# patour/distributed-membership

Hardware: AMD Instinct MI355X
Metric: simulated node-ticks/sec + achieved HBM GB/s at N=65,536 full-membership (higher is better)
Workload: dtype u8 cells (u16 escape lists) / 4-bit payload (integer)

## Files before the change

distributed-membership_amd/csrc/gm_band.h:

```cpp
#pragma once
#include "gm_device.h"
#include "gm_scaled.h"

template <int B>
struct RowMeta {
  int k;
  int snd[S_SB];
  uint32_t ebase;
  uint32_t bz;
  uint64_t evc;
  uint32_t ebase2, bz2;
  uint64_t evc2;
};

template <typename T>
__device__ __forceinline__ T gld(const T *p) {
#if __HIP_DEVICE_COMPILE__
  return *(const __attribute__((address_space(1))) T *)p;
#else
  return *p;
#endif
}
template <int B, bool UNI, bool EVC = false>
__device__ __forceinline__ RowMeta<B> row_meta(const SState &s, int r, int par, int t, size_t slab, int band,
                                               int band2 = -1) {
  RowMeta<B> m;
  const int rc = min(r, s.n - 1);
  const int32_t *ibase = par ? s.inbox[1] : s.inbox[0], *cbase = par ? s.inbox_cnt[1] : s.inbox_cnt[0];
  const int32_t *fbase = s.failed;
  const uint4 *rbase = s.brec;
  const uint64_t *ecbase = s.evcum;
  int ramp = s.ramp;
  if (UNI) asm("" : "+s"(ibase), "+s"(cbase), "+s"(fbase), "+s"(rbase), "+s"(ecbase), "+s"(ramp));
  const int32_t *ib = ibase + (size_t)rc * S_KMAX;
  const i32x4 av = gld((const i32x4 *)ib), bv = gld((const i32x4 *)(ib + 4));
  int4 a = make_int4(av.x, av.y, av.z, av.w);
  int4 b = make_int4(bv.x, bv.y, bv.z, bv.w);
  int k = gld(cbase + rc);
  int failed = gld(fbase + rc);
  const u32x4 rv = gld((const u32x4 *)(rbase + slab + rc));
  const uint4 rec = make_uint4(rv.x, rv.y, rv.z, rv.w);
  m.ebase = rec.w;
  m.bz = rec.z;
  m.evc = EVC ? gld(ecbase + (size_t)rc * s.nb + band) : 0ull;
  if (band2 >= 0) {
    const u32x4 rec2 = gld((const u32x4 *)(rbase + (size_t)band2 * s.n + rc));
    m.ebase2 = rec2.w;
    m.bz2 = rec2.z;
    m.evc2 = EVC ? gld(ecbase + (size_t)rc * s.nb + band2) : 0ull;
  }
  if (UNI) {
    asm volatile("" : "+s"(k), "+s"(failed), "+s"(a.x), "+s"(a.y), "+s"(a.z), "+s"(a.w));
    asm volatile("" : "+s"(b.x), "+s"(b.y), "+s"(b.z), "+s"(b.w));
  } else {
    asm volatile("" : "+v"(k), "+v"(failed));
  }
  m.snd[0] = a.x; m.snd[1] = a.y; m.snd[2] = a.z; m.snd[3] = a.w;
  m.snd[4] = b.x; m.snd[5] = b.y; m.snd[6] = b.z; m.snd[7] = b.w;
  m.k = (r >= s.n || failed || !s_ingroup(ramp, s.intro_until, r, t)) ? -1 : k;
  if (r >= s.n) m.ebase = m.ebase2 = 0;
  return m;
}

__device__ __forceinline__ void nib_max(u16x2 acc[8], uint32_t x0, uint32_t x1) {
  const u16x2 a = pk(x0), b = pk(x1);
  acc[0] = __builtin_elementwise_max(acc[0], a);
  acc[1] = __builtin_elementwise_max(acc[1], a << (u16x2)(4));
  acc[2] = __builtin_elementwise_max(acc[2], a << (u16x2)(8));
  acc[3] = __builtin_elementwise_max(acc[3], a << (u16x2)(12));
  acc[4] = __builtin_elementwise_max(acc[4], b);
  acc[5] = __builtin_elementwise_max(acc[5], b << (u16x2)(4));
  acc[6] = __builtin_elementwise_max(acc[6], b << (u16x2)(8));
  acc[7] = __builtin_elementwise_max(acc[7], b << (u16x2)(12));
}
__device__ __forceinline__ uint32_t nib_of(uint32_t x0, uint32_t x1, int q) {
  const uint32_t x = q < 8 ? x0 : x1;
  const int c = q & 7;
  return (x >> (16 * (c & 1) + 4 * (3 - (c >> 1)))) & 15u;
}
__device__ __forceinline__ uint32_t pesc_value(const SState &s, int pp, int band, int sn, int li, int q) {
  const uint4 rc = s.pesc_rec[pp][(size_t)band * s.n + sn];
  const uint64_t m = (uint64_t)rc.y | ((uint64_t)rc.z << 32);
  const uint32_t slot = rc.x + (uint32_t)__builtin_popcountll(m & ((1ull << li) - 1));
  return rc.x == S_PESC_NONE || slot >= s.pesc_cap ? 0u : (uint32_t)s.pesc[pp][(size_t)slot * 16 + q];
}
__device__ __forceinline__ uint32_t nib_value(uint32_t nb, const SState &s, int pp, int band, int sn, int li, int q) {
  return nb == S_NIB_ESC ? pesc_value(s, pp, band, sn, li, q) : nb ? S_NIB_H(nb) : 0u;
}

#define S_PHI 0x9E3779B9u
__device__ __forceinline__ uint32_t s_drop_pair(const SState &s, int t, int sn, int r) {
  return (uint32_t)gm_mix64(s.drop_seed ^ ((uint64_t)(uint32_t)(t - 1) << 48) ^ ((uint64_t)(uint32_t)sn << 24) ^
                            (uint64_t)(uint32_t)r);
}
__device__ __forceinline__ bool s_keep(const SState &s, int t, int sn, int r, int c, uint32_t T) {
  const uint32_t h = gm_fmix32(s_drop_pair(s, t, sn, r) ^ ((uint32_t)(c >> 1) * S_PHI));
  return ((h >> (16 * (c & 1))) & 0xFFFFu) >= T;
}
__device__ __forceinline__ constexpr int nib_pos(int q) { return 32 * (q >> 3) + 16 * (q & 1) + 4 * (3 - ((q & 7) >> 1)); }
__device__ __forceinline__ uint64_t s_keep_nibbles(const SState &s, int t, int sn, int r, int colb, uint32_t T,
                                                   bool agrp) {
  const uint32_t pair = s_drop_pair(s, t, sn, r);
  const int c = s.c0 + colb;
  if (T > 65535u) return 0;
  if (agrp) {
    const u16x2 t2 = (u16x2)((uint16_t)T);
    uint32_t kw[2] = {0u, 0u};
#pragma unroll
    for (int i = 0; i < 8; i++) {
      const uint32_t h = gm_fmix32(pair ^ ((uint32_t)((c >> 1) + i) * S_PHI));
      const u16x2 drop = pmin1(__builtin_elementwise_sub_sat(t2, pk(h)));
      kw[i >> 2] |= unpk(((u16x2)(1) - drop) * (u16x2)(0xFu << (4 * (3 - (i & 3)))));
    }
    return (uint64_t)kw[0] | ((uint64_t)kw[1] << 32);
  }
  uint64_t km = 0;
  for (int q = 0; q < 16; q++) {
    const uint32_t h = gm_fmix32(pair ^ ((uint32_t)((c + q) >> 1) * S_PHI));
    if (((h >> (16 * ((c + q) & 1))) & 0xFFFFu) >= T) km |= 0xFull << nib_pos(q);
  }
  return km;
}
__device__ __forceinline__ uint32_t nz_nibble_bits(uint32_t x) { return (x | (x >> 1) | (x >> 2) | (x >> 3)) & 0x11111111u; }

template <int B>
__device__ __forceinline__ void unit_table(const SState &s, UnitIn<B> &in) {
  constexpr int LPR = B / S_COLS_PER_LANE, Q = S_COLS_PER_LANE;
  const int li = (threadIdx.x & 63) % LPR;
  const __amdgpu_buffer_rsrc_t trs = gm_rsrc(s.table + (size_t)in.band * s.n * B, (uint32_t)(s.n * B));
  in.ta = __builtin_amdgcn_raw_buffer_load_b128(trs, (uint32_t)(in.r * B + li * Q), 0, GM_AUX_NT);
}

template <int B, bool UNI = false, bool EVC = false, bool TWO = false>
__device__ __forceinline__ void unit_load(const SState &s, int t, int band, int ub, UnitIn<B> &in,
                                          UnitIn<B> &in2, int band2) {
  constexpr int LPR = B / S_COLS_PER_LANE, RPW = 64 / LPR;
  const int sub = (threadIdx.x & 63) / LPR;
  in.band = band;
  in.r = ub * RPW + sub;
  in.msg = s.msg;
  in.tesc = (t & 1) ? s.tesc_in[0] : s.tesc_in[1];
  if (UNI) asm("" : "+s"(in.msg), "+s"(in.tesc));
  const size_t slab = (size_t)in.band * s.n;
  unit_table<B>(s, in);
  const RowMeta<B> meta = row_meta<B, UNI, EVC>(s, in.r, t & 1, t, slab, band, TWO ? band2 : -1);
#pragma unroll
  for (int j = 0; j < S_SB; j++) in.snd[j] = meta.snd[j];
  in.k = meta.k;
  in.ebase = meta.ebase;
  in.bz = meta.bz;
  in.evc = meta.evc;
  in.uni = EVC;
  if (TWO) {
    in2.band = band2;
    in2.r = in.r;
#pragma unroll
    for (int j = 0; j < S_SB; j++) in2.snd[j] = meta.snd[j];
    in2.k = meta.k;
    in2.ebase = meta.ebase2;
    in2.bz = meta.bz2;
    in2.evc = meta.evc2;
    in2.uni = EVC;
    in2.msg = in.msg;
    in2.tesc = in.tesc;
  }
}
template <int B, bool UNI = false, bool EVC = false>
__device__ __forceinline__ void unit_load(const SState &s, int t, int band, int ub, UnitIn<B> &in) {
  unit_load<B, UNI, EVC, false>(s, t, band, ub, in, in, -1);
}

template <int B, bool DROP>
__device__ __forceinline__ void unit_gather(const SState &s, int t, const UnitIn<B> &in, u32x2 m[S_SB], uint32_t &ent) {
  constexpr int LPR = B / S_COLS_PER_LANE;
  const int li = (threadIdx.x & 63) % LPR;
  ent = 0;
  if (li < (int)min(S_EW_TOT(in.ebase), (uint32_t)S_ESC_IN))
    ent = gld(in.tesc + ((size_t)in.band * s.n + in.r) * S_ESC_IN + li);
  const __amdgpu_buffer_rsrc_t prs = gm_rsrc(in.msg + (size_t)in.band * s.n * B, (uint32_t)(s.n * B));
  const uint32_t poff = (uint32_t)(((t & 1) ^ 1) * (B / 2) + li * 8);
  const int k = min(in.k, S_KMAX);
#pragma unroll
  for (int j = 0; j < S_SB; j++)
    m[j] = __builtin_amdgcn_raw_buffer_load_b64(prs, j < k ? poff + (uint32_t)in.snd[j] * B : GM_OOB, 0, 0);
}

struct RowCounts {
  uint64_t piece;
  int pf;
};
__device__ __forceinline__ RowCounts row_counts(int npres, int nfail) {
  int pf = npres | (nfail << 16);
  pf += __builtin_amdgcn_update_dpp(0, pf, 0xB1, 0xF, 0xF, false);
  pf += __builtin_amdgcn_update_dpp(0, pf, 0x4E, 0xF, 0xF, false);
  pf += __builtin_amdgcn_update_dpp(0, pf, 0x141, 0xF, 0xF, false);
  RowCounts rc;
  rc.piece = 0;
  rc.pf = 0;
#pragma unroll
  for (int c = 0; c < 8; c++) {
    const int v = __builtin_amdgcn_readlane(pf, 8 * c);
    rc.piece |= (uint64_t)(v & 0xFF) << (8 * c);
    rc.pf += v;
  }
  return rc;
}
template <int B, bool DROP>
__device__ __forceinline__ void unit_records(const SState &s, int t, const UnitIn<B> &in, bool live, uint32_t eb_out,
                                             int npres, int nfail, int nev, uint32_t evk, int nkept,
                                             const RowCounts *pre = nullptr) {
  constexpr int LPR = B / S_COLS_PER_LANE;
  constexpr int Q = S_COLS_PER_LANE;
  const int lane = threadIdx.x & 63;
  const int sub = lane / LPR, li = lane % LPR;
  const int band = in.band, r = in.r;
  const int colb = band * B + li * Q;
  const size_t slab = (size_t)band * s.n;
  if (DROP && s.mc_rdrop) {
    int v = nkept;
#pragma unroll
    for (int o = 1; o < LPR; o <<= 1) v += __shfl_xor(v, o, 64);
    if (live && li == 0 && v) atomicAdd(&s.mc_rdrop[r], (uint32_t)v);
  }
  constexpr int CH = S_CHUNK(B), LPC = CH / Q;
  int pf = npres | (nfail << 16);
  uint64_t piece = 0;
  if (LPR == 64 && LPC == 8 && pre) {
    piece = pre->piece;
    pf = pre->pf;
  } else if (LPR == 64 && LPC == 8) {
    const RowCounts rc = row_counts(npres, nfail);
    piece = rc.piece;
    pf = rc.pf;
  } else {
    int cc = npres;
#pragma unroll
    for (int o = 1; o < LPC; o <<= 1) cc += __shfl_xor(cc, o, 64);
#pragma unroll
    for (int c = 0; c < B / CH; c++) piece |= (uint64_t)(__shfl(cc, sub * LPR + LPC * c, 64) & 0xFF) << (8 * c);
#pragma unroll
    for (int o = LPR / 2; o >= 1; o >>= 1) pf += __shfl_xor(pf, o, 64);
  }
  int x = 0, tot = 0;
  if (__builtin_amdgcn_ballot_w64(nev != 0)) {
    int jr = __builtin_popcount(evk & 0x55555555u) | (__builtin_popcount(evk & 0xAAAAAAAAu) << 16);
    x = nev;
    if (LPR == 64) {
      x = dpp_scan(x);
      jr = dpp_scan(jr);
      tot = __builtin_amdgcn_readlane(x, 63);
      jr = __builtin_amdgcn_readlane(jr, 63);
    } else {
#pragma unroll
      for (int o = 1; o < LPR; o <<= 1) {
        const int y = __shfl_up(x, o, 64);
        if (li >= o) x += y;
      }
      tot = __shfl(x, sub * LPR + LPR - 1, 64);
#pragma unroll
      for (int o = LPR / 2; o >= 1; o >>= 1) jr += __shfl_xor(jr, o, 64);
    }
    if (live && li == 0 && jr) {
      const unsigned long long add = (unsigned long long)(jr & 0xFFFF) | ((unsigned long long)(jr >> 16) << 32);
      if (in.uni) s.evcum[(size_t)r * s.nb + band] = in.evc + add;
      else atomicAdd((unsigned long long *)&s.evcum[(size_t)r * s.nb + band], add);
    }
  }
  const int E = s.evs;
  uint32_t sbase = 0;
  if (live && li == 0 && tot > E) sbase = atomicAdd(s.ev_spill_cnt, (uint32_t)(tot - E));
  if (live && li == 0 && tot)
    atomicAdd(s.ev_spill_cnt + 1 + ((slab + (size_t)r) & (S_EV_STRIPES - 1)), (uint32_t)tot);
  sbase = LPR == 64 ? __builtin_amdgcn_readfirstlane(sbase) : __shfl(sbase, sub * LPR, 64);
  if (live && nev) {
    int slot = x - nev;
    uint32_t *slots = s.ev_band + ((size_t)r * s.nb + band) * E;
    for (uint32_t ek = evk; ek; ek &= ek - 1) {
      const int bit = __builtin_ctz(ek);
      const int q = bit >> 1;
      const uint32_t kind = (evk >> (2 * q)) & 3u;
      const uint32_t rec = (kind << 30) | (uint32_t)(s.c0 + colb + q + 1);
      if (slot < E) {
        slots[slot] = rec;
      } else {
        const uint32_t sp = sbase + (uint32_t)(slot - E);
        if (sp < s.ev_spill_cap) s.ev_spill[sp] = ((uint64_t)(uint32_t)r << 32) | rec;
        else atomicOr(s.err, GM_ERR_EVENTS);
      }
      slot++;
    }
  }
  if (li == 0 && r < s.n) {
    const uint32_t bc = (uint32_t)(pf & 0xFFFF) | ((uint32_t)(pf >> 16) << 11) | ((uint32_t)min(tot, 1023) << 22);
    s.brec[slab + r] = live ? make_uint4((uint32_t)piece, (uint32_t)(piece >> 32), bc, eb_out)
                            : make_uint4(0u, 0u, 0u, eb_out);
  }
}

template <int B, bool DROP>
__device__ __forceinline__ void unit_finish(const SState &s, int t, int drop_pct, const UnitIn<B> &in,
                                            const u32x2 m[S_SB], uint32_t ent, uint32_t *lds) {
  constexpr int LPR = B / S_COLS_PER_LANE;
  constexpr int RPW = 64 / LPR;
  constexpr int Q = S_COLS_PER_LANE;
  const int lane = threadIdx.x & 63;
  const int par = t & 1;
  const int sub = lane / LPR, li = lane % LPR;
  const int band = in.band, r = in.r;
  const int colb = band * B + li * Q;
  const size_t slab = (size_t)band * s.n;
  const __amdgpu_buffer_rsrc_t trs = gm_rsrc(s.table + slab * B, (uint32_t)(s.n * B));
  const __amdgpu_buffer_rsrc_t prs = gm_rsrc(s.msg + slab * B, (uint32_t)(s.n * B));
  const uint32_t toff = (uint32_t)(r * B + li * Q);
  const uint32_t poff = (uint32_t)((par ^ 1) * (B / 2) + li * 8);
  int k = in.k;
  if (k > S_KMAX) {
    if (li == 0) atomicOr(s.err, GM_ERR_INBOX);
    k = S_KMAX;
  }
  const bool live = k >= 0;
  const u32x4 ta = in.ta;
  struct {
    int snd[S_SB];
  } meta;
#pragma unroll
  for (int j = 0; j < S_SB; j++) meta.snd[j] = in.snd[j];
  int kw = 0;
  {
    const int kl = live ? k : 0;
#pragma unroll
    for (int w = 0; w < RPW; w++) kw = max(kw, __builtin_amdgcn_readlane(kl, w * LPR));
  }
  int npres = 0, nfail = 0, nev = 0;
  int nkept = 0;
  uint32_t evk = 0;
  bool esc_st = false;
  uint32_t eb_out = 0;
  if (!live && in.ebase != 0) {
    const int etot = (int)S_EW_TOT(in.ebase);
    eb_out = row_alloc<LPR>(s, par, slab, r, etot, li, lane);
    if (eb_out != 0) {
      const EscList src = esc_list(s, par ^ 1, slab, r, in.ebase), dst = esc_list(s, par, slab, r, eb_out);
      constexpr int P = LPR < S_ESC_IN ? LPR : S_ESC_IN;
      if (li < min(etot, P)) *dst.at(li) = ent;
      for (int i = P + li; i < etot; i += LPR) *dst.at(i) = *src.at(i);
    }
  }
  if (live) {
    const int32_t *ib = s.inbox[par] + (size_t)r * S_KMAX;
    u16x2 key5[8];
    {
      const uint32_t T = DROP ? s_drop_thresh(drop_pct) : 0u;
      const bool agrp = ((s.c0 + colb) & 1) == 0;
      u16x2 acc[8];
#pragma unroll
      for (int i = 0; i < 8; i++) acc[i] = (u16x2)(0);
      auto merge_list = [&](int sn, uint32_t x0, uint32_t x1) {
        if (DROP) {
          if (!(x0 | x1)) return;
          const uint64_t km = s_keep_nibbles(s, t, sn, r, colb, T, agrp);
          x0 &= (uint32_t)km;
          x1 &= (uint32_t)(km >> 32);
          if (s.mc_rdrop) nkept += __builtin_popcount(nz_nibble_bits(x0)) + __builtin_popcount(nz_nibble_bits(x1));
        }
        nib_max(acc, x0, x1);
      };
#pragma unroll
      for (int j = 0; j < S_SB; j++)
        if (j < kw) merge_list(meta.snd[j], m[j].x, m[j].y);
      for (int j = S_SB; j < k; j++) {
        const int sn = ib[j];
        const u32x2 mv = __builtin_amdgcn_raw_buffer_load_b64(prs, poff + (uint32_t)sn * B, 0, 0);
        merge_list(sn, mv.x, mv.y);
      }
      u16x2 nmax = (u16x2)(0);
#pragma unroll
      for (int i = 0; i < 8; i++) {
        const u16x2 nb = acc[i] >> (u16x2)(12);
        nmax = __builtin_elementwise_max(nmax, nb);
        key5[i] = pmin1(nb) * (u16x2)(S_NIB_BASE << 5) + nb * (u16x2)(64);
      }
      if (__builtin_elementwise_max(nmax.x, nmax.y) == S_NIB_ESC) {
#pragma unroll
        for (int i = 0; i < 8; i++) {
          const u16x2 nb = acc[i] >> (u16x2)(12);
#pragma unroll
          for (int h = 0; h < 2; h++) {
            if (nb[h] != S_NIB_ESC) continue;
            const int q = 2 * i + h;
            uint32_t kv = 0;
            for (int j = 0; j < k; j++) {
              const int sn = ib[j];
              if (DROP && !s_keep(s, t, sn, r, s.c0 + colb + q, T)) continue;
              const u32x2 mm = __builtin_amdgcn_raw_buffer_load_b64(prs, poff + (uint32_t)sn * B, 0, 0);
              kv = max(kv, nib_value(nib_of(mm.x, mm.y, q), s, par ^ 1, band, sn, li, q));
            }
            key5[i][h] = (uint16_t)(kv << 5);
          }
        }
      }
    }
    if (s.ramp && r == 0) {
#pragma unroll
      for (int q = 0; q < Q; q++) {
        const int c = s.c0 + colb + q;
        if (c >= 1 && colb + q < s.w && s_start(c) == t - 1) key5[q >> 1][q & 1] = (uint16_t)(255u << 5);
      }
    }
    const uint32_t tb4[4] = {ta.x, ta.y, ta.z, ta.w};
    u16x2 tw[8], npb = (u16x2)(0);
#pragma unroll
    for (int i = 0; i < 8; i++) {
      const u16x2 x = pk(byte_pair(tb4[i >> 1], i & 1));
      const u16x2 nz = pmin1(x);
      npb = padd(npb, nz);
      tw[i] = widen2(x, nz);
    }
    if (in.ebase != 0)
      esc_apply<LPR>(lds, lane, li, esc_list(s, par ^ 1, slab, r, in.ebase), (int)S_EW_TOT(in.ebase), ent, tw);
    u16x2 mm[8];
#pragma unroll
    for (int i = 0; i < 8; i++)
      mm[i] = __builtin_elementwise_max(__builtin_elementwise_sub_sat(tw[i], (u16x2)(63)), key5[i]);
    const int selfc = (r >= s.c0 && r < s.c0 + s.w) ? r - s.c0 - colb : -1;
    int selfapp = -1;
    if (selfc >= 0 && selfc < Q) {
      const int hb = s.hbctr[r] + 1;
      s.hbctr[r] = hb + 1;
      int tq = selfc;
      uint32_t selfcell = 0;
#pragma unroll
      for (int q = 0; q < Q; q++)
        if (q == selfc) selfcell = (unpk(mm[q >> 1]) >> (16 * (q & 1))) & 0xFFFFu;
      if (selfcell == 0) {
        if (!s.ramp) {
          atomicOr(s.err, GM_ERR_SELF);
        } else {
#pragma unroll
          for (int q = Q - 1; q >= 0; q--)
            if (q > selfc && q <= (selfc | 3) && ((unpk(mm[q >> 1]) >> (16 * (q & 1))) & 0xFFFFu)) tq = q;
          if (tq == selfc) {
            selfapp = selfc;
            const uint32_t slot = atomicAdd(s.selfadd_cnt, 1u);
            if (slot < S_SELFADD_CAP) s.selfadd[slot] = r;
            else atomicOr(s.err, GM_ERR_SELF);
            if (s.sharded) atomicOr((uint32_t *)(s.xcnt + S_XC(s, s.shard_rank, r)), S_XC_SELFAPP);
          }
        }
      }
      if (s.ramp) s.mecol[r] = s.c0 + colb + tq;
      const int h = 255 - (2 * t - (hb + s_hbase(s.ramp, s.c0 + colb + tq)));
      if (h < s.lag_hmin || h > 255) atomicOr(s.err, GM_ERR_LAG);
#pragma unroll
      for (int i = 0; i < 8; i++) {
        if ((tq >> 1) != i) continue;
        uint32_t v = unpk(mm[i]);
        const int sh = 16 * (tq & 1);
        v = (v & ~(0xFFFFu << sh)) | ((uint32_t)S_CELL(h, 0) << sh);
        mm[i] = pk(v);
      }
    }
    u16x2 np2 = (u16x2)(0), nf2 = (u16x2)(0), badv = (u16x2)(0), nmx = (u16x2)(0), amax = (u16x2)(0);
    u16x2 nwv[2] = {(u16x2)(0), (u16x2)(0)};
    uint32_t cw[8], bw[4];
    sweep_cells(mm, np2, nf2, badv, nmx, amax, nwv, cw, bw);
    int ngone = 0;
    uint32_t gmask = 0;
    if (__builtin_elementwise_max(amax.x, amax.y) >= GM_TREMOVE) {
      u16x2 ng2 = (u16x2)(0);
      uint32_t gprev = 0;
#pragma unroll
      for (int i = 0; i < 8; i++) {
        const u16x2 v = pk(cw[i]);
        const u16x2 gone = ((v & (u16x2)(31)) + (u16x2)(32 - GM_TREMOVE)) >> (u16x2)(5);
        gmask |= ((unpk(gone) & 1u) | ((unpk(gone) >> 15) & 2u)) << (2 * i);
        ng2 = padd(ng2, gone);
        const uint32_t gb = unpk(gone * (u16x2)(0xFF));
        if (i & 1) bw[i >> 1] &= ~__builtin_amdgcn_perm(gb, gprev, 0x06040200u);
        else gprev = gb;
      }
      np2 = np2 - ng2;
      ngone = (int)ng2.x + (int)ng2.y;
      badv = (u16x2)(esc_mask16(bw[0], bw[1], bw[2], bw[3]) != 0 ? 1 : 0);
    }
    esc_st = unpk(badv) != 0;
    const bool esc_row = row_any<LPR>(esc_st, sub);
    uint32_t em = 0;
    if (esc_row) {
      if (esc_st) {
        em = esc_mask16(bw[0], bw[1], bw[2], bw[3]);
        esc_park(lds, lane, cw);
      }
    }
    const bool pesc = __builtin_elementwise_max(nmx.x, nmx.y) == S_NIB_ESC;
    if (row_any<LPR>(pesc, sub)) payload_escapes<LPR>(s, par, slab, r, li, lane, sub, pesc, cw);
    nfail = (int)nf2.x + (int)nf2.y;
    npres = (int)np2.x + (int)np2.y;
    if (npres + ngone == (int)npb.x + (int)npb.y && ngone) {
      uint32_t x = gmask;
      x = (x | (x << 8)) & 0x00FF00FFu;
      x = (x | (x << 4)) & 0x0F0F0F0Fu;
      x = (x | (x << 2)) & 0x33333333u;
      x = (x | (x << 1)) & 0x55555555u;
      evk = x << 1;
      nev = __builtin_popcount(gmask);
    } else if (npres + ngone != (int)npb.x + (int)npb.y) {
      const u32x4 ra = __builtin_amdgcn_raw_buffer_load_b128(trs, toff, 0, 0);
      const uint32_t tb0[4] = {ra.x, ra.y, ra.z, ra.w};
#pragma unroll
      for (int q = 0; q < Q; q++) {
        const uint32_t before = (tb0[q >> 2] >> (8 * (q & 3))) & 0xFFu;
        const uint32_t after = (bw[q >> 2] >> (8 * (q & 3))) & 0xFFu;
        const uint32_t ev = !before ? (after && q != selfapp ? S_EV_ADD : 0u) : (!after ? S_EV_REMOVE : 0u);
        evk |= ev << (2 * q);
      }
      nev = __builtin_popcount((evk | (evk >> 1)) & 0x55555555u);
    }
    eb_out = unit_stores<B>(s, t, in, bw, unpk(nwv[0]), unpk(nwv[1]), esc_row, em, lds);
  }
  unit_records<B, DROP>(s, t, in, live, eb_out, npres, nfail, nev, evk, nkept);
}

__device__ __forceinline__ void band_reset_pools(const SState &s, int t) {
  const int S = s.esc_stripes;
  for (int i = threadIdx.x; i < S; i += 64) {
    s.tesc_cnt[((t & 1) ^ 1) * S + i] = 0;
    s.pesc_cnt[((t & 1) ^ 1) * S + i] = 0;
  }
  if (s.fb_cnt && threadIdx.x == 0) s.fb_cnt[(t & 1) ^ 1] = 0;
}

void gm_launch_selfcheck(const SState &s, hipStream_t st);
```

distributed-membership_amd/csrc/gm_band_fast.hip:

```cpp
#include "gm_band.h"

__device__ __forceinline__ int esc_bit(int q) { return ((q & 3) << 3) | (q >> 2); }
__device__ __forceinline__ int p_lanes_below(uint64_t b) {
  return (int)__builtin_amdgcn_mbcnt_hi((uint32_t)(b >> 32), __builtin_amdgcn_mbcnt_lo((uint32_t)b, 0u));
}
struct FastCell {
  uint32_t nbyte, nib, c;
  bool gone, bail;
  int dpres, dfail;
};
__device__ __forceinline__ FastCell fast_cell(const SState &s, int t, uint32_t y, uint32_t c, bool self, int hbself) {
  FastCell o;
  if (self) {
    if (c == 0) atomicOr(s.err, GM_ERR_SELF);
    const int h = 255 - (2 * t - hbself);
    if (h < s.lag_hmin || h > 255) atomicOr(s.err, GM_ERR_LAG);
    c = (uint32_t)S_CELL(h, 0) & 0xFFFFu;
  }
  const uint32_t age = c & 31u, h = c >> 5, hp = h - 2u;
  const bool pres = c != 0, stale = pres && age >= GM_TFAIL;
  o.gone = pres && age >= GM_TREMOVE;
  const bool keep = pres && !o.gone;
  const bool fits = h >= S_H4_MIN_H && !(h & 1u) && age <= S_AGE_MAX_B;
  o.nbyte = keep ? (fits ? ((((h - 224u) >> 1) << 4) | age) : S_B_ESC) : 0u;
  const bool fresh = keep && !stale;
  const bool nibok = !(hp & 1u) && hp >= S_NIB_H(1) && hp <= S_NIB_H(14);
  o.bail = fresh && !nibok;
  o.nib = fresh && nibok ? ((hp - S_NIB_BASE) >> 1) << 4 : 0u;
  o.c = c;
  const bool fpres = y >= 16u, fstale = fpres && (y & 15u) >= GM_TFAIL;
  o.dpres = (int)(pres && !o.gone) - (int)fpres;
  o.dfail = (int)stale - (int)fstale;
  return o;
}
template <int B, typename F>
__device__ __forceinline__ bool unit_fast(const SState &s, int t, const UnitIn<B> &in, const u32x2 m[S_SB],
                                          uint32_t ent, uint32_t *lds, uint32_t *park, F &&nxt) {
  static_assert(B / S_COLS_PER_LANE == 64, "the fast path takes one row per wave");
  constexpr int Q = S_COLS_PER_LANE;
  const int lane = threadIdx.x & 63, li = lane;
  const int par = t & 1;
  const int band = in.band, r = in.r;
  const int colb = band * B + li * Q;
  const size_t slab = (size_t)band * s.n;
  const int k = in.k;
  if (k > S_KMAX || s.ramp) return false;
  if (k < 0) {
    nxt();
    uint32_t eb_out = 0;
    if (in.ebase != 0) {
      const int etot = (int)S_EW_TOT(in.ebase);
      eb_out = row_alloc<64>(s, par, slab, r, etot, li, lane);
      if (eb_out != 0) {
        const EscList src = esc_list(s, par ^ 1, slab, r, in.ebase), dst = esc_list(s, par, slab, r, eb_out);
        if (li < min(etot, S_ESC_IN)) *dst.at(li) = ent;
        for (int i = S_ESC_IN + li; i < etot; i += 64) *dst.at(i) = *src.at(i);
      }
    }
    unit_records<B, false>(s, t, in, false, eb_out, 0, 0, 0, 0u, 0);
    return true;
  }
  u16x2 acc[8];
#pragma unroll
  for (int i = 0; i < 8; i++) acc[i] = (u16x2)(0);
#pragma unroll
  for (int j = 0; j < S_SB; j++)
    if (j < k) nib_max(acc, m[j].x, m[j].y);
  if (k > S_SB) {
    const __amdgpu_buffer_rsrc_t prs = gm_rsrc(s.msg + slab * B, (uint32_t)(s.n * B));
    const uint32_t poff = (uint32_t)((par ^ 1) * (B / 2) + li * 8);
    const int32_t *ib = s.inbox[par] + (size_t)r * S_KMAX;
    for (int j = S_SB; j < k; j++) {
      const int sn = ib[j];
      const u32x2 mv = __builtin_amdgcn_raw_buffer_load_b64(prs, poff + (uint32_t)sn * B, 0, 0);
      nib_max(acc, mv.x, mv.y);
    }
  }
  {
    u16x2 amx = acc[0];
#pragma unroll
    for (int i = 1; i < 8; i++) amx = __builtin_elementwise_max(amx, acc[i]);
    if (__builtin_amdgcn_ballot_w64(__builtin_elementwise_max(amx.x, amx.y) >= (uint16_t)(S_NIB_ESC << 12)))
      return false;
  }
  const uint32_t tb4[4] = {in.ta.x, in.ta.y, in.ta.z, in.ta.w};
  uint32_t bw[4], yprev = 0;
#pragma unroll
  for (int i = 0; i < 8; i++) {
    const u16x2 x = pk(byte_pair(tb4[i >> 1], i & 1));
    const u16x2 kb = (acc[i] >> (u16x2)(8)) & (u16x2)(0xF0);
    const u16x2 y = __builtin_elementwise_max(__builtin_elementwise_sub_sat(x, (u16x2)(15)), kb);
    if (i & 1) bw[i >> 1] = __builtin_amdgcn_perm(unpk(y), yprev, 0x06040200u);
    else yprev = unpk(y);
  }
  int npres = 0, nfail = 0;
  uint32_t nb[4], spm = 0;
#pragma unroll
  for (int w = 0; w < 4; w++) {
    const uint32_t v = bw[w];
    const uint32_t lo = v & 0x0F0F0F0Fu;
    const uint32_t st = (lo + 0x01010101u * (16 - GM_TFAIL)) & 0x10101010u;
    const uint32_t a15 = (lo + 0x01010101u) & 0x10101010u;
    const uint32_t hi = v & 0xF0F0F0F0u;
    const uint32_t hs = hi >> 1;
    const uint32_t pr = (hs + 0x78787878u) & 0x80808080u;
    const uint32_t g3 = (hs + 0x68686868u) & 0x80808080u;
    nfail += __builtin_popcount(st);
    npres += __builtin_popcount(pr);
    spm |= ((pr & ~g3) | (a15 << 3)) >> (7 - w);
    uint32_t st4 = st << 4;
    asm volatile("" : "+v"(st4));
    nb[w] = (hi - (pr >> 3)) & ~(st4 - st);
  }
  const int selfc = (r >= s.c0 && r < s.c0 + s.w) ? r - s.c0 - colb : -1;
  const bool selflane = selfc >= 0 && selfc < Q;
  int hbself = 0;
  if (selflane) {
    spm |= 1u << esc_bit(selfc);
    hbself = s.hbctr[r] + 1;
  }
  int ngone = 0;
  uint32_t gmask = 0, em = 0, sent = 0;
  bool sv = false, epar = true;
  const bool eslice = in.ebase != 0;
  bool quick = false;
  if (eslice && S_EW_TOT(in.ebase) <= S_ESC_IN && !__builtin_amdgcn_ballot_w64(spm != 0)) {
    const int etot = (int)S_EW_TOT(in.ebase);
    auto esc_bytes = [&](int w) {
      const uint32_t z = tb4[w] ^ (0x01010101u * S_B_ESC);
      return ~(((z & 0x7F7F7F7Fu) + 0x7F7F7F7Fu) | z) & 0x80808080u;
    };
    bool loud = false;
#pragma unroll
    for (int w = 0; w < 4; w++) loud |= ((((bw[w] >> 1) & 0x78787878u) + 0x78787878u) & esc_bytes(w)) != 0u;
    const bool ent_lane = li < etot;
    const uint32_t ev = ent_lane ? ent >> 16 : 0u;
    const uint32_t c = ev ? ev - 63u : 0u;
    const bool gone = ent_lane && (c & 31u) >= GM_TREMOVE;
    const bool fresh = ent_lane && (c & 31u) < GM_TFAIL;
    if (!__builtin_amdgcn_ballot_w64(loud || fresh)) {
      quick = true;
      int ne = 0;
#pragma unroll
      for (int w = 0; w < 4; w++) {
        const uint32_t eb = esc_bytes(w);
        static_assert(S_B_ESC == 1u, "the escape byte is restored as the detection mask's low bit");
        bw[w] |= eb >> 7;
        ne += __builtin_popcount(eb);
      }
      npres += ne;
      nfail += ne;
      const uint32_t col = ent & 0xFFFFu;
      if (__builtin_amdgcn_ballot_w64(gone)) {
        uint32_t *gw = lds;
        u32x4 *gbm = (u32x4 *)(lds + 64);
        gw[li] = 0u;
        gbm[li] = (u32x4){0u, 0u, 0u, 0u};
        lds_wave_sync();
        if (gone) {
          const uint32_t ol = col / Q, q = col % Q;
          atomicOr(gw + ol, 1u << q);
          atomicOr(lds + 64 + 4 * ol + (q >> 2), 0xFFu << (8 * (q & 3)));
        }
        lds_wave_sync();
        gmask = gw[li];
        const u32x4 bm = gbm[li];
        lds_wave_sync();
        ngone = __builtin_popcount(gmask);
        npres -= ngone;
        bw[0] &= ~bm.x;
        bw[1] &= ~bm.y;
        bw[2] &= ~bm.z;
        bw[3] &= ~bm.w;
      }
      sv = ent_lane && !gone;
      sent = col | (c << 16);
    }
  }
  const bool slow = !quick && (eslice || __builtin_amdgcn_ballot_w64(spm != 0));
  if (slow) {
    uint16_t *row16 = (uint16_t *)lds;
    u32x4 *pk4 = (u32x4 *)(park + li * 8);
    pk4[0] = (u32x4){bw[0], bw[1], bw[2], bw[3]};
    pk4[1] = (u32x4){nb[0], nb[1], nb[2], nb[3]};
    uint8_t *pall = (uint8_t *)park;
    uint8_t *pb = pall + li * 32;
    uint32_t *cor = park + S_LDS_WAVE_WORDS;
    if (eslice) cor[li] = cor[64 + li] = cor[128 + li] = 0u;
    lds_wave_sync();
    bool bail = false;
    uint32_t escm = 0;
    if (eslice) {
      const int tot = (int)S_EW_TOT(in.ebase);
      epar = tot <= 64;
      const int selfb = r - s.c0 - band * B;
      const int hbs = (selfb >= 0 && selfb < B) ? __builtin_amdgcn_readlane(hbself, selfb / Q) : 0;
      const EscList l = esc_list(s, par ^ 1, slab, r, in.ebase);
      for (int j0 = 0; j0 < tot; j0 += 64) {
        const int j = j0 + li;
        if (j < tot) {
          const uint32_t e = j < S_ESC_IN ? ent : *l.at(j);
          const int col = (int)(e & 0xFFFFu), q = col % Q, ol = col / Q;
          uint8_t *cb = pall + ol * 32 + q;
          const uint32_t y = cb[0];
          const uint32_t ev = e >> 16;
          const FastCell o = fast_cell(s, t, y, max(ev ? ev - 63u : 0u, s_widen(y)), col == selfb, hbs);
          bail |= o.bail;
          atomicOr(cor + ol, 1u << esc_bit(q));
          atomicOr(cor + 64 + ol, o.gone ? 1u << q : 0u);
          atomicAdd(cor + 128 + ol, (uint32_t)(o.dpres + o.dfail * 65536));
          cb[0] = (uint8_t)o.nbyte;
          cb[16] = (uint8_t)o.nib;
          const bool eout = o.nbyte == S_B_ESC;
          if (epar) {
            sv = eout;
            sent = (uint32_t)col | (o.c << 16);
          } else if (eout) {
            row16[col] = (uint16_t)o.c;
          }
        }
      }
      lds_wave_sync();
      escm = cor[li];
    }
    for (uint32_t mm = spm & ~escm; mm; mm &= mm - 1) {
      const int p = __builtin_ctz(mm), q = esc_cell(p);
      const uint32_t y = pb[q];
      const FastCell o = fast_cell(s, t, y, s_widen(y), q == selfc, hbself);
      bail |= o.bail;
      if (o.gone) {
        gmask |= 1u << q;
        ngone++;
      }
      if (o.nbyte == S_B_ESC) {
        em |= 1u << p;
        row16[li * Q + q] = (uint16_t)o.c;
      }
      npres += o.dpres;
      nfail += o.dfail;
      pb[q] = (uint8_t)o.nbyte;
      pb[16 + q] = (uint8_t)o.nib;
    }
    if (__builtin_amdgcn_ballot_w64(bail)) return false;
    lds_wave_sync();
    if (eslice) {
      const uint32_t ge = cor[64 + li], cd = cor[128 + li];
      gmask |= ge;
      ngone += __builtin_popcount(ge);
      const int dp = (int)(int16_t)(cd & 0xFFFFu);
      npres += dp;
      nfail += ((int)cd - dp) >> 16;
    }
    const u32x4 b0 = pk4[0], b1 = pk4[1];
    bw[0] = b0.x; bw[1] = b0.y; bw[2] = b0.z; bw[3] = b0.w;
    nb[0] = b1.x; nb[1] = b1.y; nb[2] = b1.z; nb[3] = b1.w;
    if (!epar) em = esc_mask16(bw[0], bw[1], bw[2], bw[3]);
  }
  const uint32_t ov0 = __builtin_amdgcn_perm(nb[1], nb[0], 0x01050004u) | (__builtin_amdgcn_perm(nb[1], nb[0], 0x03070206u) >> 4);
  const uint32_t ov1 = __builtin_amdgcn_perm(nb[3], nb[2], 0x01050004u) | (__builtin_amdgcn_perm(nb[3], nb[2], 0x03070206u) >> 4);
  int nev = 0;
  uint32_t evk = 0;
  const RowCounts rcnt = row_counts(npres, nfail);
  int tot = rcnt.pf & 0xFFFF;
  if (__builtin_amdgcn_ballot_w64(ngone != 0)) {
    int g = ngone;
    g += __builtin_amdgcn_update_dpp(0, g, 0xB1, 0xF, 0xF, false);
    g += __builtin_amdgcn_update_dpp(0, g, 0x4E, 0xF, 0xF, false);
    g += __builtin_amdgcn_update_dpp(0, g, 0x141, 0xF, 0xF, false);
    g += __builtin_amdgcn_update_dpp(0, g, 0x140, 0xF, 0xF, false);
    tot += __builtin_amdgcn_readlane(g, 0) + __builtin_amdgcn_readlane(g, 16) + __builtin_amdgcn_readlane(g, 32) +
           __builtin_amdgcn_readlane(g, 48);
  }
  if (tot != (int)S_BC_PRES(in.bz)) {
#pragma unroll
    for (int q = 0; q < Q; q++) {
      const uint32_t before = (tb4[q >> 2] >> (8 * (q & 3))) & 0xFFu;
      const uint32_t after = (bw[q >> 2] >> (8 * (q & 3))) & 0xFFu;
      const uint32_t ev = !before ? (after ? S_EV_ADD : 0u) : (!after ? S_EV_REMOVE : 0u);
      evk |= ev << (2 * q);
    }
    nev = __builtin_popcount((evk | (evk >> 1)) & 0x55555555u);
  } else if (ngone) {
    uint32_t x = gmask;
    x = (x | (x << 8)) & 0x00FF00FFu;
    x = (x | (x << 4)) & 0x0F0F0F0Fu;
    x = (x | (x << 2)) & 0x33333333u;
    x = (x | (x << 1)) & 0x55555555u;
    evk = x << 1;
    nev = ngone;
  }
  nxt();
  if (selflane) s.hbctr[r] = hbself + 1;
  uint32_t eb_out = unit_stores<B>(s, t, in, bw, ov0, ov1, false, 0u, lds);
  const uint64_t svb = __builtin_amdgcn_ballot_w64(sv);
  const bool emany = __builtin_amdgcn_ballot_w64(em != 0) != 0;
  if (svb || emany) {
    const int ns = __builtin_popcountll(svb);
    int etot = ns, eoff = 0;
    if (emany) {
      eoff = row_scan<64>(__builtin_popcount(em), li, lane, etot);
      etot += ns;
    }
    eb_out = row_alloc<64>(s, par, slab, r, etot, li, lane);
    if (eb_out != 0) {
      const EscList l = esc_list(s, par, slab, r, eb_out);
      if (sv) {
        *l.at(p_lanes_below(svb)) = sent;
        if ((sent >> 16) < (uint32_t)S_CELL(s.lag_hmin, 0)) atomicOr(s.err, GM_ERR_LAG);
      }
      if (emany) esc_emit(lds, lane, l, ns + eoff, em, li * Q, etot <= S_ESC_IN, s.err, s.lag_hmin);
    }
  }
  unit_records<B, false>(s, t, in, true, eb_out, npres, nfail, nev, evk, 0, &rcnt);
  return true;
}

#ifndef GM_FAST_WG
#define GM_FAST_WG 1
#endif
#ifndef GM_FAST_XS
#define GM_FAST_XS 8
#endif
#ifndef GM_FAST_MINW
#define GM_FAST_MINW 7
#endif
#ifndef GM_FAST_BPW
#define GM_FAST_BPW 2
#endif
template <int B, bool CH, int BPW>
__global__ __launch_bounds__(64 * GM_FAST_WG) __attribute__((amdgpu_waves_per_eu(GM_FAST_MINW, 8))) void gm_s_band_fast(SState s, int t, int u0, int u1) {
  if (!CH) {
    u0 = 0;
    u1 = s.n;
  }
  const int wv = GM_FAST_WG == 1 ? 0 : (int)(threadIdx.x >> 6);
  const uint32_t w = (uint32_t)((int)blockIdx.x * GM_FAST_WG + wv);
  const uint32_t q = (uint32_t)(u1 - u0 + GM_FAST_XS - 1) / GM_FAST_XS;
  const int ub = __builtin_amdgcn_readfirstlane(u0 + (int)((w % GM_FAST_XS) * q + w / GM_FAST_XS));
  if ((GM_FAST_WG > 1 && w / GM_FAST_XS >= q) || ub >= u1) return;
  constexpr int W = 2 * S_LDS_WAVE_WORDS + 192;
  __shared__ uint32_t lds_all[GM_FAST_WG * W];
  uint32_t *lds = lds_all + wv * W;
  const int b0 = (int)blockIdx.y * BPW;
  const bool two = BPW == 2 && b0 + 1 < s.nb;
  UnitIn<B> in, in2;
  unit_load<B, true, true, BPW == 2>(s, t, b0, ub, in, in2, two ? b0 + 1 : b0);
  u32x2 m[S_SB];
  uint32_t ent, ent2 = 0;
  unit_gather<B, false>(s, t, in, m, ent);
  bool issued = false;
  const bool ok = unit_fast<B>(s, t, in, m, ent, lds, lds + S_LDS_WAVE_WORDS, [&]() {
    if (two) {
      unit_table<B>(s, in2);
      unit_gather<B, false>(s, t, in2, m, ent2);
    }
    issued = true;
  });
  if (!ok && (threadIdx.x & 63) == 0) {
    const uint32_t slot = atomicAdd(&s.fb_cnt[t & 1], 1u);
    s.fb_list[slot] = make_int2(b0, ub);
  }
  if (two) {
    if (!issued) {
      unit_table<B>(s, in2);
      unit_gather<B, false>(s, t, in2, m, ent2);
    }
    lds_wave_sync();
    if (!unit_fast<B>(s, t, in2, m, ent2, lds, lds + S_LDS_WAVE_WORDS, []() {}) && (threadIdx.x & 63) == 0) {
      const uint32_t slot = atomicAdd(&s.fb_cnt[t & 1], 1u);
      s.fb_list[slot] = make_int2(b0 + 1, ub);
    }
  }
  if (ub == 0 && blockIdx.y == 0) band_reset_pools(s, t);
}
```

Measured before the change: 21.87 million.

## Transpose evcum to band-major layout and add optional wave priority hints

Changes the evcum event-counter array from row-major (row*nb+band) to band-major (band*n+row) indexing, so that adjacent waves processing consecutive rows of the same band touch contiguous memory. It also adds compile-time-gated s_setprio hints around the gather and issue segments of the fast band kernel, raising wave priority while loads are issued. The priority hints default to off (GM_FAST_PRIO=0), so only the layout change is active by default. Any other code that reads evcum with the old indexing would become inconsistent if it was not updated.

```diff
diff --git a/distributed-membership_amd/csrc/gm_band.h b/distributed-membership_amd/csrc/gm_band.h
--- a/distributed-membership_amd/csrc/gm_band.h
+++ b/distributed-membership_amd/csrc/gm_band.h
@@ -42,12 +42,12 @@
   const uint4 rec = make_uint4(rv.x, rv.y, rv.z, rv.w);
   m.ebase = rec.w;
   m.bz = rec.z;
-  m.evc = EVC ? gld(ecbase + (size_t)rc * s.nb + band) : 0ull;
+  m.evc = EVC ? gld(ecbase + slab + rc) : 0ull;
   if (band2 >= 0) {
     const u32x4 rec2 = gld((const u32x4 *)(rbase + (size_t)band2 * s.n + rc));
     m.ebase2 = rec2.w;
     m.bz2 = rec2.z;
-    m.evc2 = EVC ? gld(ecbase + (size_t)rc * s.nb + band2) : 0ull;
+    m.evc2 = EVC ? gld(ecbase + (size_t)band2 * s.n + rc) : 0ull;
   }
   if (UNI) {
     asm volatile("" : "+s"(k), "+s"(failed), "+s"(a.x), "+s"(a.y), "+s"(a.z), "+s"(a.w));
@@ -262,8 +262,8 @@
     }
     if (live && li == 0 && jr) {
       const unsigned long long add = (unsigned long long)(jr & 0xFFFF) | ((unsigned long long)(jr >> 16) << 32);
-      if (in.uni) s.evcum[(size_t)r * s.nb + band] = in.evc + add;
-      else atomicAdd((unsigned long long *)&s.evcum[(size_t)r * s.nb + band], add);
+      if (in.uni) s.evcum[slab + r] = in.evc + add;
+      else atomicAdd((unsigned long long *)&s.evcum[slab + r], add);
     }
   }
   const int E = s.evs;
diff --git a/distributed-membership_amd/csrc/gm_band_fast.hip b/distributed-membership_amd/csrc/gm_band_fast.hip
--- a/distributed-membership_amd/csrc/gm_band_fast.hip
+++ b/distributed-membership_amd/csrc/gm_band_fast.hip
@@ -1,5 +1,27 @@
 #include "gm_band.h"
 
+#ifndef GM_FAST_PRIO
+#define GM_FAST_PRIO 0
+#endif
+#ifndef GM_FAST_PRIO_LEVEL
+#define GM_FAST_PRIO_LEVEL 1
+#endif
+static_assert(GM_FAST_PRIO >= 0 && GM_FAST_PRIO <= 3 && GM_FAST_PRIO_LEVEL >= 1 && GM_FAST_PRIO_LEVEL <= 3,
+              "GM_FAST_PRIO: 0..3 segments, GM_FAST_PRIO_LEVEL: 1..3");
+template <int SEG>
+__device__ __forceinline__ void fast_prio(bool up) {
+#if GM_FAST_PRIO > 0
+  if (GM_FAST_PRIO >= SEG) {
+    if (up) __builtin_amdgcn_s_setprio(GM_FAST_PRIO_LEVEL);
+    else __builtin_amdgcn_s_setprio(0);
+  }
+#endif
+}
+__device__ __forceinline__ void fast_prio_s1(int &ub) {
+#if GM_FAST_PRIO > 0
+  asm("s_setprio %1" : "+s"(ub) : "n"(GM_FAST_PRIO_LEVEL));
+#endif
+}
 __device__ __forceinline__ int esc_bit(int q) { return ((q & 3) << 3) | (q >> 2); }
 __device__ __forceinline__ int p_lanes_below(uint64_t b) {
   return (int)__builtin_amdgcn_mbcnt_hi((uint32_t)(b >> 32), __builtin_amdgcn_mbcnt_lo((uint32_t)b, 0u));
@@ -33,7 +55,7 @@
   o.dfail = (int)stale - (int)fstale;
   return o;
 }
-template <int B, typename F>
+template <int B, int SEG, typename F>
 __device__ __forceinline__ bool unit_fast(const SState &s, int t, const UnitIn<B> &in, const u32x2 m[S_SB],
                                           uint32_t ent, uint32_t *lds, uint32_t *park, F &&nxt) {
   static_assert(B / S_COLS_PER_LANE == 64, "the fast path takes one row per wave");
@@ -46,7 +68,9 @@
   const int k = in.k;
   if (k > S_KMAX || s.ramp) return false;
   if (k < 0) {
+    fast_prio<SEG == 2 ? 2 : 4>(true);
     nxt();
+    fast_prio<SEG == 2 ? 2 : 4>(false);
     uint32_t eb_out = 0;
     if (in.ebase != 0) {
       const int etot = (int)S_EW_TOT(in.ebase);
@@ -289,6 +313,7 @@
     evk = x << 1;
     nev = ngone;
   }
+  fast_prio<SEG>(true);
   nxt();
   if (selflane) s.hbctr[r] = hbself + 1;
   uint32_t eb_out = unit_stores<B>(s, t, in, bw, ov0, ov1, false, 0u, lds);
@@ -336,7 +361,8 @@
   const int wv = GM_FAST_WG == 1 ? 0 : (int)(threadIdx.x >> 6);
   const uint32_t w = (uint32_t)((int)blockIdx.x * GM_FAST_WG + wv);
   const uint32_t q = (uint32_t)(u1 - u0 + GM_FAST_XS - 1) / GM_FAST_XS;
-  const int ub = __builtin_amdgcn_readfirstlane(u0 + (int)((w % GM_FAST_XS) * q + w / GM_FAST_XS));
+  int ub = __builtin_amdgcn_readfirstlane(u0 + (int)((w % GM_FAST_XS) * q + w / GM_FAST_XS));
+  fast_prio_s1(ub);
   if ((GM_FAST_WG > 1 && w / GM_FAST_XS >= q) || ub >= u1) return;
   constexpr int W = 2 * S_LDS_WAVE_WORDS + 192;
   __shared__ uint32_t lds_all[GM_FAST_WG * W];
@@ -348,8 +374,9 @@
   u32x2 m[S_SB];
   uint32_t ent, ent2 = 0;
   unit_gather<B, false>(s, t, in, m, ent);
+  fast_prio<1>(false);
   bool issued = false;
-  const bool ok = unit_fast<B>(s, t, in, m, ent, lds, lds + S_LDS_WAVE_WORDS, [&]() {
+  const bool ok = unit_fast<B, 2>(s, t, in, m, ent, lds, lds + S_LDS_WAVE_WORDS, [&]() {
     if (two) {
       unit_table<B>(s, in2);
       unit_gather<B, false>(s, t, in2, m, ent2);
@@ -362,11 +389,13 @@
   }
   if (two) {
     if (!issued) {
+      fast_prio<2>(true);
       unit_table<B>(s, in2);
       unit_gather<B, false>(s, t, in2, m, ent2);
     }
+    fast_prio<2>(false);
     lds_wave_sync();
-    if (!unit_fast<B>(s, t, in2, m, ent2, lds, lds + S_LDS_WAVE_WORDS, []() {}) && (threadIdx.x & 63) == 0) {
+    if (!unit_fast<B, 3>(s, t, in2, m, ent2, lds, lds + S_LDS_WAVE_WORDS, []() {}) && (threadIdx.x & 63) == 0) {
       const uint32_t slot = atomicAdd(&s.fb_cnt[t & 1], 1u);
       s.fb_list[slot] = make_int2(b0 + 1, ub);
     }
```

Measured after the change: 22.01 million (median of 6 runs). No clear change (+0.7%).
